# Storm-Tarran/LPR_381_Group_V22

Hardware: AMD Instinct MI355X
Metric: simplex pivots/sec on 4096x8192 fp64 tableau; % HBM roofline (higher is better)
Workload: dtype f64

## Files before the change

### lpr_381_group_v22_amd/csrc/overlap_kernels.hip

```cpp
#include "engine_common.hpp"
#include "select_common.hpp"

#include <new>

#include <hip/hip_ext.h>

#pragma clang fp contract(off)

#ifndef LPR_OV_DIAG
#define LPR_OV_DIAG 0
#endif

namespace lpr {

constexpr int kOvMax = 16;
constexpr int kOvNT = 256;
constexpr int kOvGroups = 64;
constexpr unsigned kOvSpinMax = 1u << 22;
constexpr int kOvDoneCopies = 32;
constexpr int kOvDoneStride = 1088;
constexpr size_t kOvFlagWords = (size_t)(kOvDoneCopies + 1) * kOvDoneStride;
#ifndef LPR_OV_TILE_ROWS
#define LPR_OV_TILE_ROWS 32
#endif
constexpr int kOvTileRows = LPR_OV_TILE_ROWS;
#ifndef LPR_OV_WAVE_HANDOFF
#define LPR_OV_WAVE_HANDOFF 1
#endif
constexpr bool kOvWaveHandoff = LPR_OV_WAVE_HANDOFF != 0;
constexpr int kOvWPG = kOvNT / 64;
constexpr int kOvParts = kOvGroups * kOvWPG;

struct OvCtl {
    int32_t status;
    int32_t pending;
    int32_t kdone;
    int32_t slot;
    int32_t cur;
    int32_t sweep;
    int32_t r[kOvMax];
    int32_t error;
    int32_t head_xcc;
    int64_t staged;
    int64_t applied;
    int64_t max_iter;
    int64_t log_cap;
};

struct OvBuffers {
    double* Tb[2];
    double* prow;
    double* fcol;
    double* zrow;
    double* bvec;
    ZPart* zparts;
    double* rparts;
    unsigned long long* gran;
    unsigned long long* xgran;
    unsigned long long* hx;
    unsigned* tileq;
    unsigned* sflag;
    unsigned long long* dbg;
    OvCtl* ctl;
    unsigned* bar;
    int32_t* basis;
    int32_t* log;
};

constexpr int kOvStampsPerPivot = 12;
constexpr int kOvStampPivots = 64;
constexpr size_t kOvDbgLaunch = (size_t)kOvStampPivots * kOvStampsPerPivot + 8;
constexpr size_t kOvDbgWords = kOvDbgLaunch + 64;

__global__ __launch_bounds__(1024) void k_ov_prologue(const double* __restrict__ T, int ld, int R,
                                                      int C, double* __restrict__ zrow,
                                                      double* __restrict__ bvec0,
                                                      ZPart* __restrict__ bank, int G,
                                                      unsigned long long* gbank,
                                                      unsigned epoch,
                                                      unsigned long long* gran_all,
                                                      unsigned long long* __restrict__ xgran,
                                                      unsigned* __restrict__ bar,
                                                      unsigned* __restrict__ tileq,
                                                      unsigned long long* __restrict__ hx,
                                                      unsigned* __restrict__ sflag) {
    __shared__ double lds_v[16];
    __shared__ int lds_i[16];
    const int tid = threadIdx.x, nt = blockDim.x;
    for (int k = tid; k < 9 * kOvParts; k += nt) gran_all[k] = 0ull;
    for (int k = tid; k < kOvGroups; k += nt) xgran[k] = 0ull;
    if (tid < 4) bar[tid] = 0u;
    if (tid < 2) tileq[tid] = 0u;
    if (tid == 0) *hx = 0ull;
    if (tid < 4) sflag[tid] = 0u;
    if (tid < kOvDoneCopies) sflag[(size_t)(tid + 1) * kOvDoneStride] = 0u;
    __syncthreads();
    Cand c;
    c.v = 0.0;
    c.i = -1;
    for (int j = tid; j < ld; j += nt) {
        const double v = T[j];
        zrow[j] = v;
        if (j < C - 1 && v < c.v) {
            c.v = v;
            c.i = j;
        }
    }
    c = block_cand_min(c, lds_v, lds_i);
    if (tid < G) {
        const double v = (tid == 0) ? c.v : 0.0;
        const int i = (tid == 0) ? c.i : -1;
        bank[tid].v = v;
        bank[tid].i = i;
    }
    const int nparts = kOvWaveHandoff ? G * kOvWPG : G;
    if (tid < nparts) {
        const double v = (tid == 0) ? c.v : 0.0;
        const int i = (tid == 0) ? c.i : -1;
        const unsigned long long e = (unsigned long long)epoch << 32;
        gbank[tid * 3 + 0] = e | (unsigned)__double2loint(v);
        gbank[tid * 3 + 1] = e | (unsigned)__double2hiint(v);
        gbank[tid * 3 + 2] = e | (unsigned)i;
    }
    for (int i = tid; i < R; i += nt) bvec0[i] = T[(size_t)i * ld + (C - 1)];
}

__device__ __forceinline__ double xld(const double* p) {
    return __hip_atomic_load(p, __ATOMIC_RELAXED, __HIP_MEMORY_SCOPE_AGENT);
}
__device__ __forceinline__ void xst(double* p, double v) {
    __hip_atomic_store(p, v, __ATOMIC_RELAXED, __HIP_MEMORY_SCOPE_AGENT);
}
__device__ __forceinline__ int xld(const int* p) {
    return __hip_atomic_load(p, __ATOMIC_RELAXED, __HIP_MEMORY_SCOPE_AGENT);
}
__device__ __forceinline__ void xst(int* p, int v) {
    __hip_atomic_store(p, v, __ATOMIC_RELAXED, __HIP_MEMORY_SCOPE_AGENT);
}

__device__ __forceinline__ void hst(double* p, double v, bool l2) {
    if (l2) __hip_atomic_store(p, v, __ATOMIC_RELAXED, __HIP_MEMORY_SCOPE_WORKGROUP);
    else __hip_atomic_store(p, v, __ATOMIC_RELAXED, __HIP_MEMORY_SCOPE_AGENT);
}
__device__ __forceinline__ void hst(unsigned long long* p, unsigned long long v, bool l2) {
    if (l2) __hip_atomic_store(p, v, __ATOMIC_RELAXED, __HIP_MEMORY_SCOPE_WORKGROUP);
    else __hip_atomic_store(p, v, __ATOMIC_RELAXED, __HIP_MEMORY_SCOPE_AGENT);
}
__device__ __forceinline__ unsigned ov_xcc_id() {
    unsigned v;
    asm volatile("s_getreg_b32 %0, hwreg(HW_REG_XCC_ID)" : "=s"(v));
    return v & 0xfu;
}
__device__ __forceinline__ unsigned long long ov_now() { return __builtin_amdgcn_s_memrealtime(); }

__device__ __forceinline__ double ov_rl(double v, int k) {
    const int lo = __builtin_amdgcn_readlane(__double2loint(v), k);
    const int hi = __builtin_amdgcn_readlane(__double2hiint(v), k);
    return __hiloint2double(hi, lo);
}

__device__ __forceinline__ double ov_bitsel(unsigned mask, int t, double a, double b) {
    int m, lo, hi;
    asm("v_bfe_i32 %0, %1, %2, 1" : "=v"(m) : "v"(mask), "s"(t));
    asm("v_bfi_b32 %0, %1, %2, %3" : "=v"(lo) : "v"(m), "s"(__double2loint(a)), "v"(__double2loint(b)));
    asm("v_bfi_b32 %0, %1, %2, %3" : "=v"(hi) : "v"(m), "s"(__double2hiint(a)), "v"(__double2hiint(b)));
    return __hiloint2double(hi, lo);
}

__device__ __forceinline__ Cand ov_cand_min_sel(Cand a, Cand b) {
    const bool take = (b.i >= 0) & ((a.i < 0) | (b.v < a.v) | ((b.v == a.v) & (b.i < a.i)));
    Cand r;
    r.v = take ? b.v : a.v;
    r.i = take ? b.i : a.i;
    return r;
}

template <int CTRL, int ROW_MASK>
__device__ __forceinline__ Cand ov_dpp_min(Cand c) {
// ... 864 lines not shown
            {
                const double dn[3] = {wr, w.x, w.y}, dd[3] = {p, p, p};
                ieee_div_n<3>(dn, dd, dq);
            }
            const double prhs = dq[0];
            if (lane == q - 1) {
                prhsNv = prhs;
                rNv = r;
            }
            if (have_i && i_first == r) maskN |= 1u << (q - 1);
            Cand n;
            n.v = 0.0;
            n.i = -1;
            if (have_c) {
                const int j = 2 * c2_first;
                double2 pq;
                pq.x = (j < C) ? dq[1] : 0.0;
                pq.y = (j + 1 < C) ? dq[2] : 0.0;
#pragma unroll
                for (int t = 0; t < kOvMax; ++t)
                    if (t == q - 1) myp[t] = pq;
                hst(&prowN[(size_t)(q - 1) * ld + j], pq.x, l2);
                hst(&prowN[(size_t)(q - 1) * ld + j + 1], pq.y, l2);
                const double mxp = f0 * pq.x;
                const double myp2 = f0 * pq.y;
                myz.x = myz.x - mxp;
                myz.y = myz.y - myp2;
                zrow2[c2_first] = myz;
                if (j < C - 1 && myz.x < n.v) {
                    n.v = myz.x;
                    n.i = j;
                }
                if (j + 1 < C - 1 && myz.y < n.v) {
                    n.v = myz.y;
                    n.i = j + 1;
                }
            }
            for (int c2 = c2_first + G * nt; c2 < ld2; c2 += G * nt) {
                double2 ww = Tin2[(size_t)r * ld2 + c2];
                double2 z = zrow2[c2];
#pragma unroll
                for (int t = 0; t < kOvMax; ++t) {
                    if (t < kb) {
                        const double2 ps = prowA2[(size_t)t * ld2 + c2];
                        if ((ra >> t) & 1u) {
                            ww = ps;
                        } else {
                            const double f = ov_rl(fv, t);
                            const double px = f * ps.x;
                            const double py = f * ps.y;
                            ww.x = ww.x - px;
                            ww.y = ww.y - py;
                        }
                    }
                }
#pragma unroll
                for (int t = 0; t < kOvMax; ++t) {
                    if (t < q - 1) {
                        double2 ps;
                        ps.x = prowN[(size_t)t * ld + 2 * c2];
                        ps.y = prowN[(size_t)t * ld + 2 * c2 + 1];
                        if ((rn >> t) & 1u) {
                            ww = ps;
                        } else {
                            const double f = ov_rl(fv, kOvMax + t);
                            const double px = f * ps.x;
                            const double py = f * ps.y;
                            ww.x = ww.x - px;
                            ww.y = ww.y - py;
                        }
                    }
                }
                const int j = 2 * c2;
                double2 pq;
                pq.x = (j < C) ? ieee_div(ww.x, p) : 0.0;
                pq.y = (j + 1 < C) ? ieee_div(ww.y, p) : 0.0;
                hst(&prowN[(size_t)(q - 1) * ld + j], pq.x, l2);
                hst(&prowN[(size_t)(q - 1) * ld + j + 1], pq.y, l2);
                const double mxp = f0 * pq.x;
                const double myp2 = f0 * pq.y;
                z.x = z.x - mxp;
                z.y = z.y - myp2;
                zrow2[c2] = z;
                if (j < C - 1 && z.x < n.v) {
                    n.v = z.x;
                    n.i = j;
                }
                if (j + 1 < C - 1 && z.y < n.v) {
                    n.v = z.y;
                    n.i = j + 1;
                }
            }
            if (have_i) {
                const double prod = cq * prhs;
                myb = (i_first == r) ? prhs : myb - prod;
                hst(&bnew[i_first], myb, l2);
            }
            for (int i = i_first + G * nt; i < R; i += G * nt) {
                const double prod = colq[i] * prhs;
                hst(&bnew[i], (i == r) ? prhs : bprev[i] - prod, l2);
            }
            OV_STAMP(q, 9);
            if (lead && tid == 0) {
                co->r[q - 1] = r;
                B.basis[r - 1] = e;
                if (pidx < log_cap) {
                    B.log[2 * pidx] = r;
                    B.log[2 * pidx + 1] = e;
                }
            }
            count = q;
            OV_STAMP(q, 10);
            if (kOvWaveHandoff)
                ov_publish_wave_min(n, B.gran + ((size_t)((pidx + 1) & 1) * kOvParts + g * kOvWPG +
                                                 tid / kWave) * 3,
                                    (unsigned)(2 * (pidx + 1) + 1), l2 && q < K);
            else
                ov_publish_min(n, lds_v, lds_i,
                               B.gran + ((size_t)((pidx + 1) & 1) * kOvParts + g) * 3,
                               (unsigned)(2 * (pidx + 1) + 1), l2 && q < K);
            OV_STAMP(q, 11);
        }
    }
#undef OV_STAMP

    if (STAMP && stamp) B.dbg[kOvDbgLaunch + 8 * ((staged0 / 16) & 7) + 2] = ov_now();
    if (lead && tid == 0) {
        const bool staged_now = (status == kRunning && pend_in == kRunning);
        if (wait_sweeps > 0 && !staged_now) {
            unsigned spins = 0;
            while (__hip_atomic_load(B.sflag, __ATOMIC_RELAXED, __HIP_MEMORY_SCOPE_AGENT) <
                   (unsigned)wait_sweeps) {
                if (++spins > kOvSpinMax) {
                    err = 1;
                    break;
                }
                __builtin_amdgcn_s_sleep(2);
            }
        }
        co->status = err ? LPR_DEVICE_ERROR : status_out;
        co->pending = pend_out;
        co->kdone = staged_now ? count : 0;
        co->slot = staged_now ? (sa ^ 1) : sa;
        co->staged = staged0 + (staged_now ? count : 0);
        co->max_iter = mx;
        co->log_cap = log_cap;
        co->error = err | ci->error;
        co->head_xcc = l2 ? (int)my_xcc : (staging ? -1 : ci->head_xcc);
        B.bar[lp ^ 1] = 0u;
        if (wait_sweeps >= 0) {
            const int ks = (status == kRunning) ? ci->kdone : 0;
            co->applied = ci->applied + ks;
            co->cur = (ks > 0) ? (ci->cur ^ 1) : ci->cur;
            co->sweep = ci->sweep ^ 1;
        }
        if (solo) {
            B.tileq[1] = 0u;
            co->applied = ci->applied;
            co->cur = ci->cur;
            co->sweep = ci->sweep;
        }
    }
    if (heads_done >= 0) {
        asm volatile("s_waitcnt vmcnt(0)" ::: "memory");
        __syncthreads();
        if (tid == 0) {
            __builtin_amdgcn_fence(__ATOMIC_RELEASE, "agent");
            const unsigned old = __hip_atomic_fetch_add(B.sflag + 2, 1u, __ATOMIC_RELAXED,
                                                        __HIP_MEMORY_SCOPE_AGENT);
            s_pick[0] = (old + 1u == (unsigned)G) ? 1 : 0;
            if (s_pick[0])
                __hip_atomic_store(B.sflag + 2, 0u, __ATOMIC_RELAXED, __HIP_MEMORY_SCOPE_AGENT);
        }
        __syncthreads();
        if (s_pick[0]) {
            if (tid <= kOvDoneCopies)
                __hip_atomic_store(tid == 0 ? B.sflag + 1 : B.sflag + (size_t)tid * kOvDoneStride,
                                   (unsigned)heads_done, __ATOMIC_RELAXED,
                                   __HIP_MEMORY_SCOPE_AGENT);
            if (STAMP && tid == 0)
                B.dbg[kOvDbgLaunch + 8 * ((staged0 / 16) & 7) + 3] = ov_now();
        }
    }
}

template <typename T>
__device__ __forceinline__ T ov_ld_stream(const T* p) {
    return __builtin_nontemporal_load(p);
}

typedef double ov_v2d __attribute__((ext_vector_type(2)));

template <int TR>
__device__ __forceinline__ void ov_chunk(ov_v2d (&x)[TR], const ov_v2d (&p)[kOvMax],
                                         const double* __restrict__ fci, int Rp) {
    if (LPR_OV_DIAG & 1) return;
    constexpr int kSteps = (LPR_OV_DIAG & 4) ? kOvMax / 2 : kOvMax;
    double fn[TR];
#pragma unroll
    for (int k = 0; k < TR; ++k) fn[k] = fci[k];
#pragma unroll
    for (int s = 0; s < kSteps; ++s) {
        double f[TR];
#pragma unroll
        for (int k = 0; k < TR; ++k) f[k] = fn[k];
        if (s + 1 < kSteps) {
            size_t off = (size_t)(s + 1) * Rp;
            asm volatile("" : "+s"(off) : "s"(f[0]));
#pragma unroll
            for (int k = 0; k < TR; ++k) fn[k] = fci[off + k];
        }
#pragma unroll
        for (int k = 0; k < TR; ++k) {
            const double px = f[k] * p[s].x;
            const double py = f[k] * p[s].y;
            x[k].x = x[k].x - px;
            x[k].y = x[k].y - py;
        }
#pragma unroll
        for (int k = 0; k < TR; ++k) asm volatile("" : "+v"(x[k]));
    }
}

template <int TR, bool INPLACE>
__device__ __forceinline__ void ov_rows_load(ov_v2d (&x)[TR], const ov_v2d* src, int ld2) {
#pragma unroll
    for (int k = 0; k < TR; ++k)
        x[k] = (INPLACE || (LPR_OV_DIAG & 8)) ? src[(size_t)k * ld2]
                                              : ov_ld_stream(&src[(size_t)k * ld2]);
}

template <int TR, bool INPLACE>
__device__ __forceinline__ void ov_rows_store(const ov_v2d (&x)[TR], ov_v2d* dst, int ld2,
                                              unsigned skip) {
#pragma unroll
    for (int k = 0; k < TR; ++k) {
        if ((skip >> k) & 1u) continue;
        if (INPLACE || (LPR_OV_DIAG & 8)) dst[(size_t)k * ld2] = x[k];
        else if (LPR_OV_DIAG & 64)
            asm volatile("global_store_dwordx4 %0, %1, off sc0 sc1 nt" ::"v"(&dst[(size_t)k * ld2]),
                         "v"(x[k])
                         : "memory");
        else if (LPR_OV_DIAG & 128)
            asm volatile("global_store_dwordx4 %0, %1, off sc1 nt" ::"v"(&dst[(size_t)k * ld2]),
                         "v"(x[k])
                         : "memory");
        else __builtin_nontemporal_store(x[k], &dst[(size_t)k * ld2]);
    }
}

template <int TR, bool DB, bool INPLACE, int TROWS = kOvTileRows>
__device__ __forceinline__ void ov_one_tile(const OvBuffers& B, const OvCtl* ci,
                                            const double* __restrict__ fc,
                                            const ov_v2d* __restrict__ prow2, int tb, int ld,
                                            int R, int Rp, int K, int cur, int unit = TROWS,
                                            int off = 0) {
    typedef ov_v2d v2d;
    const int ld2 = ld >> 1;
    const int nct = (ld2 + kOvNT - 1) / kOvNT;
    const int nrt = (R + unit - 1) / unit;
    if (LPR_OV_DIAG & 16) {
        const int per = (nct * nrt + 7) / 8;
        tb = (tb % 8) * per + tb / 8;
    }
    int ct = tb % nct, rt = tb / nct;
    if (LPR_OV_DIAG & 32) {
        rt = tb % nrt;
        ct = tb / nrt;
        if (ct >= nct) return;
    }
    if (rt >= nrt) return;
    if (ci->sweep & 1) {
        ct = nct - 1 - ct;
        rt = nrt - 1 - rt;
    }
    const int c2 = ct * kOvNT + threadIdx.x;
    if (c2 >= ld2) return;
    const v2d* Tin2 = reinterpret_cast<const v2d*>(B.Tb[cur]);
    v2d* Tout2 = reinterpret_cast<v2d*>(B.Tb[INPLACE ? cur : (cur ^ 1)]);
    v2d p[kOvMax];
#pragma unroll
    for (int s = 0; s < kOvMax; ++s) {
        if (LPR_OV_DIAG & 2) p[s] = v2d{(double)c2, (double)s};
        else p[s] = prow2[(size_t)s * ld2 + c2];
    }
    const int ibase = rt * unit + off;
    const int iend = min(R, ibase + TROWS);
    if (ibase >= R) return;

    if (K == kOvMax && iend - ibase == TROWS) {
        unsigned long long prmask = 0ull;
#pragma unroll
        for (int s = 0; s < kOvMax; ++s) {
            const int r = ci->r[s];
            if (r >= ibase && r < iend) prmask |= 1ull << (r - ibase);
        }
        const v2d* src = Tin2 + (size_t)ibase * ld2 + c2;
        v2d* dst = Tout2 + (size_t)ibase * ld2 + c2;
        const size_t step = (size_t)TR * ld2;
        if (DB) {
            v2d xa[TR], xb[TR];
            ov_rows_load<TR, INPLACE>(xa, src, ld2);
#pragma unroll 1
            for (int j = 0; j < TROWS; j += 2 * TR) {
                ov_rows_load<TR, INPLACE>(xb, src + step, ld2);
                ov_chunk<TR>(xa, p, fc + ibase + j, Rp);
                ov_rows_store<TR, INPLACE>(xa, dst, ld2, (unsigned)(prmask >> j));
                if (j + 2 * TR < TROWS) ov_rows_load<TR, INPLACE>(xa, src + 2 * step, ld2);
                ov_chunk<TR>(xb, p, fc + ibase + j + TR, Rp);
                ov_rows_store<TR, INPLACE>(xb, dst + step, ld2, (unsigned)(prmask >> (j + TR)));
                src += 2 * step;
                dst += 2 * step;
            }
        } else {
#pragma unroll 1
            for (int j = 0; j < TROWS; j += TR) {
                v2d x[TR];
                ov_rows_load<TR, INPLACE>(x, src, ld2);
                ov_chunk<TR>(x, p, fc + ibase + j, Rp);
                ov_rows_store<TR, INPLACE>(x, dst, ld2, (unsigned)(prmask >> j));
                src += step;
                dst += step;
            }
        }
        if (prmask) {
#pragma unroll
            for (int s0 = 0; s0 < kOvMax; ++s0) {
                const int i = ci->r[s0];
                if (i < ibase || i >= iend) continue;
                bool again = false;
#pragma unroll
                for (int s1 = s0 + 1; s1 < kOvMax; ++s1) again = again || (ci->r[s1] == i);
                if (again) continue;
                v2d t = p[s0];
#pragma unroll
                for (int s1 = s0 + 1; s1 < kOvMax; ++s1) {
                    const double f = fc[(size_t)s1 * Rp + i];
                    const double px = f * p[s1].x;
                    const double py = f * p[s1].y;
                    t.x = t.x - px;
                    t.y = t.y - py;
                }
                v2d* d = &Tout2[(size_t)i * ld2 + c2];
                if (INPLACE) *d = t;
                else __builtin_nontemporal_store(t, d);
            }
        }
        return;
    }
    int rr[kOvMax];
#pragma unroll
    for (int s = 0; s < kOvMax; ++s) rr[s] = (s < K) ? ci->r[s] : -1;
    for (int i0 = ibase; i0 < iend; i0 += TR) {
        v2d x[TR];
#pragma unroll
        for (int k = 0; k < TR; ++k) {
            const int i = i0 + k;
            if (i < iend) {
                const v2d* src = &Tin2[(size_t)i * ld2 + c2];
                x[k] = INPLACE ? *src : ov_ld_stream(src);
            }
        }
#pragma unroll
        for (int k = 0; k < TR; ++k) {
            const int i = i0 + k;
            if (i < iend) {
                v2d t = x[k];
#pragma unroll
                for (int s = 0; s < kOvMax; ++s) {
                    if (s < K) {
                        if (i == rr[s]) {
                            t = p[s];
                        } else {
                            const double f = fc[(size_t)s * Rp + i];
                            const double px = f * p[s].x;
                            const double py = f * p[s].y;
                            t.x = t.x - px;
                            t.y = t.y - py;
                        }
                    }
                }
                v2d* dst = &Tout2[(size_t)i * ld2 + c2];
                if (INPLACE) *dst = t;
                else __builtin_nontemporal_store(t, dst);
            }
        }
    }
}

template <int TR, bool DB, bool INPLACE, int TROWS = kOvTileRows>
__device__ __forceinline__ void ov_tiles(const OvBuffers& B, const double* __restrict__ fcol,
                                         const double* __restrict__ prow, int ld, int R, int Rp,
                                         int G, int lp, int static_tile, int avoid,
                                         bool write_ctl = true, int sweeps_done = -1,
                                         int wait_heads = -1, int hint_xcc = -1) {
    static_assert(TROWS % TR == 0 && (!DB || TROWS % (2 * TR) == 0) && TROWS <= 64,
                  "tile rows: a multiple of the chunks in flight, and one bit each in prmask");
    __shared__ int s_tile;
    const bool first_wg = ((int)blockIdx.x == G);
    if (first_wg && threadIdx.x == 0 && sweeps_done >= 0)
        __hip_atomic_store(B.sflag, (unsigned)sweeps_done, __ATOMIC_RELAXED,
                           __HIP_MEMORY_SCOPE_AGENT);
    if (first_wg && threadIdx.x == 0 && !INPLACE && B.dbg)
        B.dbg[kOvDbgLaunch + 8 * (wait_heads > 0 ? (wait_heads & 7)
                                                  : (int)((B.ctl[lp].applied / 16 + 1) & 7)) + 4] = ov_now();
    if (wait_heads > 0) {
        if (threadIdx.x == 0) {
            int go = 0;
            const unsigned* word =
                B.sflag + (size_t)(1 + ((int)blockIdx.x & (kOvDoneCopies - 1))) * kOvDoneStride;
            auto ready = [&]() {
                return __hip_atomic_load(word, __ATOMIC_RELAXED, __HIP_MEMORY_SCOPE_AGENT) >=
                       (unsigned)wait_heads;
            };
            if (!first_wg && hint_xcc >= 0 && (int)ov_xcc_id() == hint_xcc) {
                go = 0;
            } else if (ready()) {
                go = 1;
            } else {
                go = -1;
                for (unsigned spins = 0; spins < kOvSpinMax; ++spins) {
                    __builtin_amdgcn_s_sleep(8);
                    if (ready()) {
                        go = 1;
                        break;
                    }
                }
                if (go < 0)
                    __hip_atomic_store(B.sflag + 3, 1u, __ATOMIC_RELAXED, __HIP_MEMORY_SCOPE_AGENT);
            }
            s_tile = go;
        }
        __syncthreads();
        const int go = s_tile;
        __syncthreads();
        if (go <= 0) return;
        if (first_wg && threadIdx.x == 0 && B.dbg) B.dbg[kOvDbgLaunch + 8 * (wait_heads & 7) + 5] = ov_now();
        if (!(hint_xcc >= 0 && (int)ov_xcc_id() == hint_xcc))
            __builtin_amdgcn_fence(__ATOMIC_ACQUIRE, "agent");
        __builtin_amdgcn_s_dcache_inv();
    }
    const OvCtl* ci = B.ctl + lp;
    const int K = (ci->status == kRunning) ? ci->kdone : 0;
    const int cur = ci->cur;
    if (first_wg && threadIdx.x == 0) {
        OvCtl* co = B.ctl + (lp ^ 1);
        if (write_ctl) {
            co->applied = ci->applied + K;
            co->cur = (K > 0 && !INPLACE) ? (cur ^ 1) : cur;
            co->sweep = ci->sweep ^ 1;
        }
        B.tileq[lp ^ 1] = 0u;
        if (INPLACE) {
            co->status = ci->status;
            co->pending = ci->pending;
            co->kdone = 0;
            co->slot = ci->slot;
            co->staged = ci->staged;
            co->max_iter = ci->max_iter;
            co->log_cap = ci->log_cap;
            co->error = ci->error;
            co->head_xcc = ci->head_xcc;
            B.bar[lp ^ 1] = 0u;
        }
    }
    if (K <= 0) return;
    const int sa = ci->slot;
    const double* __restrict__ fc = fcol + (size_t)sa * kOvMax * Rp;
    const ov_v2d* __restrict__ prow2 =
        reinterpret_cast<const ov_v2d*>(prow + (size_t)sa * kOvMax * ld);
    if (static_tile >= 0) {
        ov_one_tile<TR, DB, INPLACE, TROWS>(B, ci, fc, prow2, static_tile, ld, R, Rp, K, cur);
        return;
    }
    const int ld2 = ld >> 1;
    const int ntiles = ((ld2 + kOvNT - 1) / kOvNT) * ((R + TROWS - 1) / TROWS);
    constexpr bool kHalfTail = (TROWS / 2) % TR == 0 && TROWS == kOvTileRows && (LPR_OV_DIAG & 256) == 0;
#ifndef LPR_OV_TAIL_DIV
#define LPR_OV_TAIL_DIV 4
#endif
    const int tsplit = kHalfTail ? (ntiles - ntiles / LPR_OV_TAIL_DIV) : ntiles;
    const int qtiles = tsplit + 2 * (ntiles - tsplit);
    const bool heads_beside = !INPLACE && avoid > 0 && ci->status == kRunning &&
                              ci->pending == kRunning;
    const unsigned my_xcc = ov_xcc_id();
    if (heads_beside && avoid > 1 && ci->head_xcc == (int)my_xcc) return;
    const unsigned xepoch = (unsigned)(ci->staged + 1);
    for (;;) {
        if (threadIdx.x == 0) {
            int tile = -1;
            if (heads_beside) {
                const unsigned long long v =
                    __hip_atomic_load(B.hx, __ATOMIC_RELAXED, __HIP_MEMORY_SCOPE_AGENT);
                if ((unsigned)(v >> 32) == xepoch && ((unsigned)v & 0x1ffu) == (0x100u | my_xcc))
                    tile = qtiles;
            }
            if (tile < 0)
                tile = (int)__hip_atomic_fetch_add(B.tileq + lp, 1u, __ATOMIC_RELAXED,
                                                   __HIP_MEMORY_SCOPE_AGENT);
            s_tile = tile;
        }
        __syncthreads();
        const int tile = s_tile;
        __syncthreads();
        if (tile >= qtiles) return;
        if (tile < tsplit) {
            ov_one_tile<TR, DB, INPLACE, TROWS>(B, ci, fc, prow2, tile, ld, R, Rp, K, cur);
        } else {
            const int u = tile - tsplit;
            ov_one_tile<TR, false, INPLACE, TROWS / 2>(B, ci, fc, prow2, tsplit + (u >> 1), ld, R, Rp,
                                                       K, cur, TROWS, (u & 1) * (TROWS / 2));
        }
    }
}

template <int TR, bool DB>
__global__ __launch_bounds__(kOvNT) void k_ov_step(const OvBuffers B,
                                                   const double* __restrict__ fcol_ro,
                                                   const double* __restrict__ prow_ro, int ld,
                                                   int R, int C, int Rp, int K, int G, int lp) {
    if ((int)blockIdx.x < G)
        ov_heads<kOvNT>(B, ld, R, C, Rp, K, G, lp, false);
    else
        ov_tiles<TR, DB, false>(B, fcol_ro, prow_ro, ld, R, Rp, G, lp, (int)blockIdx.x - G, 0);
}

template <int NT, bool STAMP>
__global__ __launch_bounds__(NT) void k_ov2_heads(const OvBuffers B, int ld, int R, int C, int Rp,
                                                  int K, int G, int lp, int spread, int no_l2,
                                                  int wait_sweeps, int heads_done) {
    ov_heads_rich<NT, STAMP>(B, ld, R, C, Rp, K, G, lp, false, spread, no_l2, wait_sweeps,
                             heads_done);
}



template <int TR, bool DB>
__global__ __launch_bounds__(kOvNT) void k_ov2_sweep(const OvBuffers B,
                                                     const double* __restrict__ fcol_ro,
                                                     const double* __restrict__ prow_ro, int ld,
                                                     int R, int Rp, int lp, int avoid,
                                                     int write_ctl, int sweeps_done,
                                                     int wait_heads, int hint_xcc) {
    ov_tiles<TR, DB, false>(B, fcol_ro, prow_ro, ld, R, Rp, 0, lp, -1, avoid, write_ctl != 0,
                            sweeps_done, wait_heads, hint_xcc);
}

template <int NT, bool STAMP>
__global__ __launch_bounds__(NT) void k_ov_heads(const OvBuffers B, int ld, int R, int C, int Rp,
                                                 int K, int G, int spread, int no_l2) {
    ov_heads_rich<NT, STAMP>(B, ld, R, C, Rp, K, G, 0, true, spread, no_l2, -1);
}

template <int TR, bool DB, int TROWS = kOvTileRows>
__global__ __launch_bounds__(kOvNT) void k_ov_sweep(const OvBuffers B,
                                                    const double* __restrict__ fcol_ro,
                                                    const double* __restrict__ prow_ro, int ld,
                                                    int R, int Rp) {
    ov_tiles<TR, DB, true, TROWS>(B, fcol_ro, prow_ro, ld, R, Rp, 0, 1, (int)blockIdx.x, 0);
}

}

#ifndef LPR_OV_KERNELS_ONLY

struct lpr_overlap_ctx {
    int rows = 0, ld = 0, Rp = 0;
    lpr::OvBuffers b{};
    lpr::OvCtl* h_ctl = nullptr;
    double* h_z = nullptr;
    double* T2 = nullptr;
    hipStream_t hstream = nullptr;
    hipEvent_t ev_h[2] = {nullptr, nullptr}, ev_s[2] = {nullptr, nullptr};
    int ev_idx = 0;
    int steps = 0;
    hipEvent_t last_sweep = nullptr;
    unsigned* h_flags = nullptr;
    int head_xcc_hint = -1;
    bool batch_first = true;
};

namespace lpr {

struct OvPoll {
    int32_t status, pending, kdone, cur, error;
    int64_t applied;
    double z[2];
};

int ov_max_pivots() { return kOvMax; }

void ov_release(lpr_tableau* t) {
    lpr_overlap_ctx* c = static_cast<lpr_overlap_ctx*>(t->ov);
    if (!c) return;
    if (c->hstream) {
        hipStreamSynchronize(c->hstream);
        hipStreamDestroy(c->hstream);
        for (int k = 0; k < 2; ++k) {
            hipEventDestroy(c->ev_h[k]);
            hipEventDestroy(c->ev_s[k]);
        }
    }
    hipFree(c->T2);
    hipFree(c->b.prow);
    hipFree(c->b.fcol);
    hipFree(c->b.zrow);
    hipFree(c->b.bvec);
    hipFree(c->b.zparts);
    hipFree(c->b.rparts);
    hipFree(c->b.gran);
    hipFree(c->b.xgran);
    hipFree(c->b.hx);
    hipFree(c->b.tileq);
    hipFree(c->b.sflag);
    hipFree(c->b.dbg);
    hipFree(c->b.ctl);
    hipFree(c->b.bar);
    if (c->h_ctl) hipHostFree(c->h_ctl);
    if (c->h_z) hipHostFree(c->h_z);
    if (c->h_flags) hipHostFree(c->h_flags);
    delete c;
    t->ov = nullptr;
}

int ov_ensure(lpr_tableau* t, bool second_buffer) {
    lpr_overlap_ctx* c = static_cast<lpr_overlap_ctx*>(t->ov);
    if (c && c->rows == t->rows && c->ld == t->ld && (c->T2 || !second_buffer))
        return LPR_OK_OPTIMAL;
    ov_release(t);
    c = new (std::nothrow) lpr_overlap_ctx();
    if (!c) return LPR_OUT_OF_MEMORY;
    c->rows = t->rows;
    c->ld = t->ld;
    c->Rp = align_up(t->rows, 16);
    hipError_t err = hipSuccess;
    auto chk = [&](hipError_t x) { if (err == hipSuccess) err = x; };
    const size_t D = sizeof(double);
    const size_t tbytes = (size_t)t->rows * t->ld * D;
    if (second_buffer) chk(hipMalloc(&c->T2, tbytes));
    chk(hipMalloc(&c->b.prow, (size_t)2 * kOvMax * c->ld * D));
    chk(hipMalloc(&c->b.fcol, (size_t)2 * kOvMax * c->Rp * D));
    chk(hipMalloc(&c->b.zrow, (size_t)c->ld * D));
    chk(hipMalloc(&c->b.bvec, (size_t)2 * c->Rp * D));
    chk(hipMalloc(&c->b.zparts, (size_t)2 * kOvGroups * sizeof(ZPart)));
    chk(hipMalloc(&c->b.rparts, (size_t)(3 * kOvGroups + 1) * sizeof(double)));
    chk(hipMalloc(&c->b.gran, (size_t)9 * kOvParts * sizeof(unsigned long long)));
    chk(hipMalloc(&c->b.xgran, (size_t)kOvGroups * sizeof(unsigned long long)));
    chk(hipMalloc(&c->b.dbg, kOvDbgWords * sizeof(unsigned long long)));
    chk(hipMalloc(&c->b.hx, 2 * sizeof(unsigned long long)));
    chk(hipMalloc(&c->b.tileq, 4 * sizeof(unsigned)));
    chk(hipMalloc(&c->b.sflag, kOvFlagWords * sizeof(unsigned)));
    chk(hipMalloc(&c->b.ctl, 2 * sizeof(OvCtl)));
    chk(hipMalloc(&c->b.bar, 4 * sizeof(unsigned)));
    chk(hipHostMalloc(&c->h_ctl, 2 * sizeof(OvCtl)));
    chk(hipHostMalloc(&c->h_z, 2 * sizeof(double)));
    chk(hipHostMalloc(&c->h_flags, 4 * sizeof(unsigned)));
    t->ov = c;
    if (err != hipSuccess) {
        set_error("overlapped-pivot scratch allocation failed: %s", hipGetErrorString(err));
        ov_release(t);
        return err == hipErrorOutOfMemory ? LPR_OUT_OF_MEMORY : LPR_DEVICE_ERROR;
    }
    hipStream_t s = t->eng->stream;
    if (c->T2) LPR_HIP(hipMemsetAsync(c->T2, 0, tbytes, s));
    LPR_HIP(hipMemsetAsync(c->b.prow, 0, (size_t)2 * kOvMax * c->ld * D, s));
    LPR_HIP(hipMemsetAsync(c->b.fcol, 0, (size_t)2 * kOvMax * c->Rp * D, s));
    LPR_HIP(hipMemsetAsync(c->b.zrow, 0, (size_t)c->ld * D, s));
    LPR_HIP(hipMemsetAsync(c->b.bvec, 0, (size_t)2 * c->Rp * D, s));
    LPR_HIP(hipMemsetAsync(c->b.zparts, 0, (size_t)2 * kOvGroups * sizeof(ZPart), s));
    LPR_HIP(hipMemsetAsync(c->b.dbg, 0, kOvDbgWords * sizeof(unsigned long long), s));
    LPR_HIP(hipMemsetAsync(c->b.sflag, 0, kOvFlagWords * sizeof(unsigned), s));
    std::memset(c->h_ctl, 0, 2 * sizeof(OvCtl));
    std::memset(c->h_flags, 0, 4 * sizeof(unsigned));
    return LPR_OK_OPTIMAL;
}

static int ov_tile_code(int tr) {
    switch (tr) {
        case 0x04: case 0x10: case 0x24: case 0x28: return tr;
        default: return 0x08;
    }
}

static int ov_spread(int G, int flags) { return ((flags & 2) || G > 32) ? 1 : 8; }

static int ov_sweep_grid(const lpr_tableau* t, int ntiles) {
    const int cap = 4 * (t->eng->num_cus > 0 ? t->eng->num_cus : 256);
    return ntiles < cap ? (ntiles > 0 ? ntiles : 1) : cap;
}

static int ov_groups(const lpr_tableau* t) {
    int g = (t->ld / 2 + kOvNT - 1) / kOvNT;
    if (g < 1) g = 1;
    if (g > kOvGroups) g = kOvGroups;
    return g;
}

int ov_begin(lpr_tableau* t, int64_t iter, int64_t max_iter) {
    lpr_overlap_ctx* c = static_cast<lpr_overlap_ctx*>(t->ov);
    hipStream_t s = t->eng->stream;
    c->b.Tb[0] = t->T;
    c->b.Tb[1] = c->T2;
    c->b.basis = t->basis;
    c->b.log = t->log;
    OvCtl* h = c->h_ctl;
    std::memset(h, 0, 2 * sizeof(OvCtl));
    h[0].status = kRunning;
    h[0].pending = kRunning;
    h[0].staged = iter;
    h[0].applied = iter;
    h[0].max_iter = max_iter;
    h[0].log_cap = t->log_cap;
    h[0].head_xcc = -1;
    h[1] = h[0];
    LPR_HIP(hipMemcpyAsync(c->b.ctl, h, 2 * sizeof(OvCtl), hipMemcpyHostToDevice, s));
    hipLaunchKernelGGL(k_ov_prologue, dim3(1), dim3(1024), 0, s, t->T, t->ld, t->rows, t->cols,
                       c->b.zrow, c->b.bvec + (size_t)(iter & 1) * c->Rp,
                       c->b.zparts + (iter & 1) * kOvGroups, ov_groups(t),
                       c->b.gran + (size_t)(iter & 1) * 3 * kOvParts, (unsigned)(2 * iter + 1),
                       c->b.gran, c->b.xgran, c->b.bar, c->b.tileq, c->b.hx, c->b.sflag);
    LPR_HIP(hipGetLastError());
    return LPR_OK_OPTIMAL;
}

int ov_set_log(lpr_tableau* t, int parity) {
    lpr_overlap_ctx* c = static_cast<lpr_overlap_ctx*>(t->ov);
    c->b.log = t->log;
    c->h_ctl[0].log_cap = t->log_cap;
    LPR_HIP(hipMemcpyAsync(&c->b.ctl[parity].log_cap, &c->h_ctl[0].log_cap, sizeof(int64_t),
                           hipMemcpyHostToDevice, t->eng->stream));
    LPR_HIP(hipStreamSynchronize(t->eng->stream));
    return LPR_OK_OPTIMAL;
}

void ov_launch_step(lpr_tableau* t, int K, int tr, int lp) {
    lpr_overlap_ctx* c = static_cast<lpr_overlap_ctx*>(t->ov);
    hipStream_t s = t->eng->stream;
    const int G = ov_groups(t);
    const int ld2 = t->ld / 2;
    const int nct = (ld2 + kOvNT - 1) / kOvNT;
    const int nrt = (t->rows + kOvTileRows - 1) / kOvTileRows;
    const dim3 grid(G + nct * nrt), blk(kOvNT);
#define LPR_OV_STEP(TR, DB)                                                                      \
    hipLaunchKernelGGL((k_ov_step<TR, DB>), grid, blk, 0, s, c->b, c->b.fcol, c->b.prow, t->ld,   \
                       t->rows, t->cols, c->Rp, K, G, lp)
    if (tr >= 16) LPR_OV_STEP(16, false);
    else if (tr >= 8) LPR_OV_STEP(8, false);
    else LPR_OV_STEP(4, false);
#undef LPR_OV_STEP
}

void ov_launch_heads(lpr_tableau* t, int K, int flags) {
    lpr_overlap_ctx* c = static_cast<lpr_overlap_ctx*>(t->ov);
    const int G = ov_groups(t);
    const int spread = ov_spread(G, flags);
    const int no_l2 = (flags & 6) ? 1 : 0;
    hipStream_t s = t->eng->stream;
    if (flags & 1)
        hipLaunchKernelGGL((k_ov_heads<kOvNT, true>), dim3(G * spread), dim3(kOvNT), 0, s, c->b,
                           t->ld, t->rows, t->cols, c->Rp, K, G, spread, no_l2);
    else
        hipLaunchKernelGGL((k_ov_heads<kOvNT, false>), dim3(G * spread), dim3(kOvNT), 0, s, c->b,
                           t->ld, t->rows, t->cols, c->Rp, K, G, spread, no_l2);
}

void ov_launch_sweep(lpr_tableau* t, int tr) {
    lpr_overlap_ctx* c = static_cast<lpr_overlap_ctx*>(t->ov);
    hipStream_t s = t->eng->stream;
    const int nct = (t->ld / 2 + kOvNT - 1) / kOvNT;
    const int nrt = (t->rows + kOvTileRows - 1) / kOvTileRows;
    const int cus = t->eng->num_cus > 0 ? t->eng->num_cus : 256;
    if (nct * nrt < 2 * cus && ov_tile_code(tr) == 0x08) {
        const int nrt8 = (t->rows + 7) / 8;
        hipLaunchKernelGGL((k_ov_sweep<8, false, 8>), dim3(nct * nrt8), dim3(kOvNT), 0, s, c->b,
                           c->b.fcol, c->b.prow, t->ld, t->rows, c->Rp);
        return;
    }
    const dim3 grid(nct * nrt), blk(kOvNT);
#define LPR_OV_SWEEP(TR, DB)                                                                     \
    hipLaunchKernelGGL((k_ov_sweep<TR, DB>), grid, blk, 0, s, c->b, c->b.fcol, c->b.prow, t->ld,  \
                       t->rows, c->Rp)
    switch (ov_tile_code(tr)) {
        case 0x04: LPR_OV_SWEEP(4, false); break;
        case 0x10: LPR_OV_SWEEP(16, false); break;
        case 0x24: LPR_OV_SWEEP(4, true); break;
        case 0x28: LPR_OV_SWEEP(8, true); break;
        default: LPR_OV_SWEEP(8, false); break;
    }
#undef LPR_OV_SWEEP
}

int ov2_begin(lpr_tableau* t) {
    lpr_overlap_ctx* c = static_cast<lpr_overlap_ctx*>(t->ov);
    if (!c->hstream) {
        int lo = 0, hi = 0;
        LPR_HIP(hipDeviceGetStreamPriorityRange(&lo, &hi));
        LPR_HIP(hipStreamCreateWithPriority(&c->hstream, hipStreamNonBlocking, hi));
        for (int k = 0; k < 2; ++k) {
            LPR_HIP(hipEventCreateWithFlags(&c->ev_h[k], hipEventDisableTiming));
            LPR_HIP(hipEventCreateWithFlags(&c->ev_s[k], hipEventDisableTiming));
        }
    }
    c->ev_idx = 0;
    c->steps = 0;
    c->batch_first = true;
    LPR_HIP(hipEventRecord(c->ev_s[1], t->eng->stream));
    LPR_HIP(hipEventRecord(c->ev_h[1], c->hstream));
    c->last_sweep = c->ev_s[1];
    LPR_HIP(hipStreamWaitEvent(c->hstream, c->ev_s[1], 0));
    return LPR_OK_OPTIMAL;
}

int ov2_launch_step(lpr_tableau* t, int K, int tr, int lp, int flags, hipEvent_t ev_start,
                    hipEvent_t ev_stop) {
    lpr_overlap_ctx* c = static_cast<lpr_overlap_ctx*>(t->ov);
    hipStream_t S = t->eng->stream, H = c->hstream;
    const int cur = c->ev_idx, prev = cur ^ 1;
    const bool by_event = (flags & 32) == 0;
    const int wait_sweeps = by_event ? -1 : c->steps;
    const bool sweep_dev = (flags & 64) != 0 && !c->batch_first && c->steps >= 2 &&
                           c->head_xcc_hint >= 0;
    const int heads_done = (flags & 64) ? c->steps + 1 : -1;
    if (by_event) LPR_HIP(hipStreamWaitEvent(H, c->last_sweep, 0));
    if (!sweep_dev) LPR_HIP(hipStreamWaitEvent(S, c->ev_h[prev], 0));
    const int G = ov_groups(t);
    const int spread = ov_spread(G, flags);
    const int no_l2 = (flags & 6) ? 1 : 0;
    if (flags & 1)
        hipExtLaunchKernelGGL((k_ov2_heads<kOvNT, true>), dim3(G * spread), dim3(kOvNT), 0, H,
                              nullptr, c->ev_h[cur], 0, c->b, t->ld, t->rows, t->cols, c->Rp, K, G,
                              lp, spread, no_l2, wait_sweeps, heads_done);
    else
        hipExtLaunchKernelGGL((k_ov2_heads<kOvNT, false>), dim3(G * spread), dim3(kOvNT), 0, H,
                              nullptr, c->ev_h[cur], 0, c->b, t->ld, t->rows, t->cols, c->Rp, K, G,
                              lp, spread, no_l2, wait_sweeps, heads_done);
    const int nct = (t->ld / 2 + kOvNT - 1) / kOvNT;
    const int nrt = (t->rows + kOvTileRows - 1) / kOvTileRows;
    const dim3 grid(ov_sweep_grid(t, nct * nrt)), blk(kOvNT);
    const int avoid = (flags & (2 | 4 | 8)) ? 0 : ((flags & 16) ? 1 : 2);
    hipEvent_t sweep_done = ev_stop ? ev_stop : c->ev_s[cur];
#define LPR_OV2_SWEEP(TR, DB)                                                                     \
    hipExtLaunchKernelGGL((k_ov2_sweep<TR, DB>), grid, blk, 0, S, ev_start, sweep_done, 0, c->b,   \
                          c->b.fcol, c->b.prow, t->ld, t->rows, c->Rp, lp, avoid, by_event ? 1 : 0, \
                          by_event ? -1 : c->steps, sweep_dev ? c->steps : -1, c->head_xcc_hint)
    switch (ov_tile_code(tr)) {
        case 0x04: LPR_OV2_SWEEP(4, false); break;
        case 0x10: LPR_OV2_SWEEP(16, false); break;
        case 0x24: LPR_OV2_SWEEP(4, true); break;
        case 0x28: LPR_OV2_SWEEP(8, true); break;
        default: LPR_OV2_SWEEP(8, false); break;
    }
#undef LPR_OV2_SWEEP
    c->last_sweep = sweep_done;
    c->steps += 1;
    c->ev_idx = prev;
    c->batch_first = false;
    return LPR_OK_OPTIMAL;
}

int ov2_join(lpr_tableau* t) {
    lpr_overlap_ctx* c = static_cast<lpr_overlap_ctx*>(t->ov);
    LPR_HIP(hipStreamWaitEvent(t->eng->stream, c->ev_h[c->ev_idx ^ 1], 0));
    c->batch_first = true;
    return LPR_OK_OPTIMAL;
}

int ov_poll(lpr_tableau* t, int parity, OvPoll* out) {
    lpr_overlap_ctx* c = static_cast<lpr_overlap_ctx*>(t->ov);
    hipStream_t s = t->eng->stream;
    LPR_HIP(hipMemcpyAsync(c->h_ctl, c->b.ctl, 2 * sizeof(OvCtl), hipMemcpyDeviceToHost, s));
    LPR_HIP(hipMemcpyAsync(&c->h_z[0], c->b.bvec, sizeof(double), hipMemcpyDeviceToHost, s));
    LPR_HIP(hipMemcpyAsync(&c->h_z[1], c->b.bvec + c->Rp, sizeof(double), hipMemcpyDeviceToHost,
                           s));
    LPR_HIP(hipMemcpyAsync(c->h_flags, c->b.sflag, 4 * sizeof(unsigned), hipMemcpyDeviceToHost, s));
    LPR_HIP(hipStreamSynchronize(s));
    const OvCtl& h = c->h_ctl[parity];
    c->head_xcc_hint = h.head_xcc;
    out->status = h.status;
    out->pending = h.pending;
    out->kdone = h.kdone;
    out->cur = h.cur;
    out->error = h.error | (c->h_flags[3] ? 1 : 0);
    out->applied = h.applied;
    out->z[0] = c->h_z[0];
    out->z[1] = c->h_z[1];
    return LPR_OK_OPTIMAL;
}

int ov_read_stamps(lpr_tableau* t, uint64_t* out, int64_t cap, int64_t* count) {
    lpr_overlap_ctx* c = static_cast<lpr_overlap_ctx*>(t->ov);
    if (!c) {
        *count = 0;
        return LPR_OK_OPTIMAL;
    }
    int64_t n = (int64_t)kOvDbgWords;
    if (n > cap) n = cap;
    *count = n;
    if (n > 0 && out) {
        LPR_HIP(hipStreamSynchronize(t->eng->stream));
        LPR_HIP(hipMemcpy(out, c->b.dbg, (size_t)n * sizeof(uint64_t), hipMemcpyDeviceToHost));
    }
    return LPR_OK_OPTIMAL;
}

void ov_adopt_buffer(lpr_tableau* t, int cur) {
    lpr_overlap_ctx* c = static_cast<lpr_overlap_ctx*>(t->ov);
    if (cur == 1) {
        double* tmp = t->T;
        t->T = c->T2;
        c->T2 = tmp;
    }
}

}
#endif
```

Measured before the change: 90840.

## Use cacheable loads/stores on boundary tiles to keep sweep data in Infinity Cache

The sweep kernel now uses plain (cacheable) loads for the first tiles of each sweep and plain stores for the last tiles, sized to about 64 MB. Because successive sweeps alternate direction, data just written stays resident in the last-level cache for the next sweep's start. Sweep direction is now toggled only when pivots are applied, and is kept across polls so the serpentine order survives batch boundaries. This trades nontemporal streaming on those tiles for possible cache pollution and adds template instantiations, which may raise code size.

```diff
diff --git a/lpr_381_group_v22_amd/csrc/overlap_kernels.hip b/lpr_381_group_v22_amd/csrc/overlap_kernels.hip
--- a/lpr_381_group_v22_amd/csrc/overlap_kernels.hip
+++ b/lpr_381_group_v22_amd/csrc/overlap_kernels.hip
@@ -24,6 +24,10 @@
 #define LPR_OV_TILE_ROWS 32
 #endif
 constexpr int kOvTileRows = LPR_OV_TILE_ROWS;
+#ifndef LPR_OV_IC_MB
+#define LPR_OV_IC_MB 64
+#endif
+constexpr int kOvIcMB = LPR_OV_IC_MB;
 #ifndef LPR_OV_WAVE_HANDOFF
 #define LPR_OV_WAVE_HANDOFF 1
 #endif
@@ -1194,7 +1198,7 @@
             const int ks = (status == kRunning) ? ci->kdone : 0;
             co->applied = ci->applied + ks;
             co->cur = (ks > 0) ? (ci->cur ^ 1) : ci->cur;
-            co->sweep = ci->sweep ^ 1;
+            co->sweep = ci->sweep ^ (ks > 0 ? 1 : 0);
         }
         if (solo) {
             B.tileq[1] = 0u;
@@ -1264,21 +1268,21 @@
     }
 }
 
-template <int TR, bool INPLACE>
+template <int TR, bool PLAIN>
 __device__ __forceinline__ void ov_rows_load(ov_v2d (&x)[TR], const ov_v2d* src, int ld2) {
 #pragma unroll
     for (int k = 0; k < TR; ++k)
-        x[k] = (INPLACE || (LPR_OV_DIAG & 8)) ? src[(size_t)k * ld2]
-                                              : ov_ld_stream(&src[(size_t)k * ld2]);
-}
-
-template <int TR, bool INPLACE>
+        x[k] = (PLAIN || (LPR_OV_DIAG & 8)) ? src[(size_t)k * ld2]
+                                            : ov_ld_stream(&src[(size_t)k * ld2]);
+}
+
+template <int TR, bool PLAIN>
 __device__ __forceinline__ void ov_rows_store(const ov_v2d (&x)[TR], ov_v2d* dst, int ld2,
                                               unsigned skip) {
 #pragma unroll
     for (int k = 0; k < TR; ++k) {
         if ((skip >> k) & 1u) continue;
-        if (INPLACE || (LPR_OV_DIAG & 8)) dst[(size_t)k * ld2] = x[k];
+        if (PLAIN || (LPR_OV_DIAG & 8)) dst[(size_t)k * ld2] = x[k];
         else if (LPR_OV_DIAG & 64)
             asm volatile("global_store_dwordx4 %0, %1, off sc0 sc1 nt" ::"v"(&dst[(size_t)k * ld2]),
                          "v"(x[k])
@@ -1291,7 +1295,7 @@
     }
 }
 
-template <int TR, bool DB, bool INPLACE, int TROWS = kOvTileRows>
+template <int TR, bool DB, bool INPLACE, int TROWS = kOvTileRows, int POL = 0>
 __device__ __forceinline__ void ov_one_tile(const OvBuffers& B, const OvCtl* ci,
                                             const double* __restrict__ fc,
                                             const ov_v2d* __restrict__ prow2, int tb, int ld,
@@ -1312,7 +1316,7 @@
         if (ct >= nct) return;
     }
     if (rt >= nrt) return;
-    if (ci->sweep & 1) {
+    if ((ci->sweep & 1) && !(LPR_OV_DIAG & 512)) {
         ct = nct - 1 - ct;
         rt = nrt - 1 - rt;
     }
@@ -1340,17 +1344,18 @@
         const v2d* src = Tin2 + (size_t)ibase * ld2 + c2;
         v2d* dst = Tout2 + (size_t)ibase * ld2 + c2;
         const size_t step = (size_t)TR * ld2;
+        constexpr bool kPlainLd = INPLACE || (POL & 1), kPlainSt = INPLACE || (POL & 2);
         if (DB) {
             v2d xa[TR], xb[TR];
-            ov_rows_load<TR, INPLACE>(xa, src, ld2);
+            ov_rows_load<TR, kPlainLd>(xa, src, ld2);
 #pragma unroll 1
             for (int j = 0; j < TROWS; j += 2 * TR) {
-                ov_rows_load<TR, INPLACE>(xb, src + step, ld2);
+                ov_rows_load<TR, kPlainLd>(xb, src + step, ld2);
                 ov_chunk<TR>(xa, p, fc + ibase + j, Rp);
-                ov_rows_store<TR, INPLACE>(xa, dst, ld2, (unsigned)(prmask >> j));
-                if (j + 2 * TR < TROWS) ov_rows_load<TR, INPLACE>(xa, src + 2 * step, ld2);
+                ov_rows_store<TR, kPlainSt>(xa, dst, ld2, (unsigned)(prmask >> j));
+                if (j + 2 * TR < TROWS) ov_rows_load<TR, kPlainLd>(xa, src + 2 * step, ld2);
                 ov_chunk<TR>(xb, p, fc + ibase + j + TR, Rp);
-                ov_rows_store<TR, INPLACE>(xb, dst + step, ld2, (unsigned)(prmask >> (j + TR)));
+                ov_rows_store<TR, kPlainSt>(xb, dst + step, ld2, (unsigned)(prmask >> (j + TR)));
                 src += 2 * step;
                 dst += 2 * step;
             }
@@ -1358,9 +1363,9 @@
 #pragma unroll 1
             for (int j = 0; j < TROWS; j += TR) {
                 v2d x[TR];
-                ov_rows_load<TR, INPLACE>(x, src, ld2);
+                ov_rows_load<TR, kPlainLd>(x, src, ld2);
                 ov_chunk<TR>(x, p, fc + ibase + j, Rp);
-                ov_rows_store<TR, INPLACE>(x, dst, ld2, (unsigned)(prmask >> j));
+                ov_rows_store<TR, kPlainSt>(x, dst, ld2, (unsigned)(prmask >> j));
                 src += step;
                 dst += step;
             }
@@ -1435,7 +1440,8 @@
                                          const double* __restrict__ prow, int ld, int R, int Rp,
                                          int G, int lp, int static_tile, int avoid,
                                          bool write_ctl = true, int sweeps_done = -1,
-                                         int wait_heads = -1, int hint_xcc = -1) {
+                                         int wait_heads = -1, int hint_xcc = -1,
+                                         int ic_tiles = 0) {
     static_assert(TROWS % TR == 0 && (!DB || TROWS % (2 * TR) == 0) && TROWS <= 64,
                   "tile rows: a multiple of the chunks in flight, and one bit each in prmask");
     __shared__ int s_tile;
@@ -1490,7 +1496,7 @@
         if (write_ctl) {
             co->applied = ci->applied + K;
             co->cur = (K > 0 && !INPLACE) ? (cur ^ 1) : cur;
-            co->sweep = ci->sweep ^ 1;
+            co->sweep = ci->sweep ^ (K > 0 ? 1 : 0);
         }
         B.tileq[lp ^ 1] = 0u;
         if (INPLACE) {
@@ -1546,12 +1552,29 @@
         const int tile = s_tile;
         __syncthreads();
         if (tile >= qtiles) return;
+        const int at = tile < tsplit ? tile : tsplit + ((tile - tsplit) >> 1);
+        const int pol = (at < ic_tiles ? 1 : 0) | (at >= ntiles - ic_tiles ? 2 : 0);
         if (tile < tsplit) {
-            ov_one_tile<TR, DB, INPLACE, TROWS>(B, ci, fc, prow2, tile, ld, R, Rp, K, cur);
+#define LPR_OV_FULL(P) ov_one_tile<TR, DB, INPLACE, TROWS, P>(B, ci, fc, prow2, tile, ld, R, Rp, K, cur)
+            switch (pol) {
+                case 1: LPR_OV_FULL(1); break;
+                case 2: LPR_OV_FULL(2); break;
+                case 3: LPR_OV_FULL(3); break;
+                default: LPR_OV_FULL(0); break;
+            }
+#undef LPR_OV_FULL
         } else {
             const int u = tile - tsplit;
-            ov_one_tile<TR, false, INPLACE, TROWS / 2>(B, ci, fc, prow2, tsplit + (u >> 1), ld, R, Rp,
-                                                       K, cur, TROWS, (u & 1) * (TROWS / 2));
+#define LPR_OV_HALF(P)                                                                             \
+    ov_one_tile<TR, false, INPLACE, TROWS / 2, P>(B, ci, fc, prow2, tsplit + (u >> 1), ld, R, Rp, \
+                                                  K, cur, TROWS, (u & 1) * (TROWS / 2))
+            switch (pol) {
+                case 1: LPR_OV_HALF(1); break;
+                case 2: LPR_OV_HALF(2); break;
+                case 3: LPR_OV_HALF(3); break;
+                default: LPR_OV_HALF(0); break;
+            }
+#undef LPR_OV_HALF
         }
     }
 }
@@ -1583,9 +1606,9 @@
                                                      const double* __restrict__ prow_ro, int ld,
                                                      int R, int Rp, int lp, int avoid,
                                                      int write_ctl, int sweeps_done,
-                                                     int wait_heads, int hint_xcc) {
+                                                     int wait_heads, int hint_xcc, int ic_tiles) {
     ov_tiles<TR, DB, false>(B, fcol_ro, prow_ro, ld, R, Rp, 0, lp, -1, avoid, write_ctl != 0,
-                            sweeps_done, wait_heads, hint_xcc);
+                            sweeps_done, wait_heads, hint_xcc, ic_tiles);
 }
 
 template <int NT, bool STAMP>
@@ -1619,6 +1642,7 @@
     hipEvent_t last_sweep = nullptr;
     unsigned* h_flags = nullptr;
     int head_xcc_hint = -1;
+    int sweep_dir = 0;
     bool batch_first = true;
 };
 
@@ -1754,6 +1778,7 @@
     h[0].max_iter = max_iter;
     h[0].log_cap = t->log_cap;
     h[0].head_xcc = -1;
+    h[0].sweep = c->sweep_dir;
     h[1] = h[0];
     LPR_HIP(hipMemcpyAsync(c->b.ctl, h, 2 * sizeof(OvCtl), hipMemcpyHostToDevice, s));
     hipLaunchKernelGGL(k_ov_prologue, dim3(1), dim3(1024), 0, s, t->T, t->ld, t->rows, t->cols,
@@ -1881,10 +1906,13 @@
     const dim3 grid(ov_sweep_grid(t, nct * nrt)), blk(kOvNT);
     const int avoid = (flags & (2 | 4 | 8)) ? 0 : ((flags & 16) ? 1 : 2);
     hipEvent_t sweep_done = ev_stop ? ev_stop : c->ev_s[cur];
+    const int ic_tiles =
+        (flags & 128) ? 0 : (int)(((size_t)kOvIcMB << 20) / ((size_t)kOvTileRows * kOvNT * 16));
 #define LPR_OV2_SWEEP(TR, DB)                                                                     \
     hipExtLaunchKernelGGL((k_ov2_sweep<TR, DB>), grid, blk, 0, S, ev_start, sweep_done, 0, c->b,   \
                           c->b.fcol, c->b.prow, t->ld, t->rows, c->Rp, lp, avoid, by_event ? 1 : 0, \
-                          by_event ? -1 : c->steps, sweep_dev ? c->steps : -1, c->head_xcc_hint)
+                          by_event ? -1 : c->steps, sweep_dev ? c->steps : -1, c->head_xcc_hint,    \
+                          ic_tiles)
     switch (ov_tile_code(tr)) {
         case 0x04: LPR_OV2_SWEEP(4, false); break;
         case 0x10: LPR_OV2_SWEEP(16, false); break;
@@ -1918,6 +1946,7 @@
     LPR_HIP(hipStreamSynchronize(s));
     const OvCtl& h = c->h_ctl[parity];
     c->head_xcc_hint = h.head_xcc;
+    c->sweep_dir = h.sweep & 1;
     out->status = h.status;
     out->pending = h.pending;
     out->kdone = h.kdone;
```

After: 94050, median of 6. 3.5% higher.
